# askerlee/AdaFace-dev

Hardware: AMD Instinct MI355X
Metric: denoise-steps/sec SD-1.5 U-Net 512px bs=4/GPU (higher is better)
Workload: dtype f16

## Files before the change

adaface-dev_amd/csrc/af_gemm3.hip:

```cpp
#include <stdlib.h>

#include <algorithm>

#include "af_common.h"

int af_gemm_n_major(int M, int N, int K, int cin);

namespace {

struct Gemm3Dev {
  const half_t* a1;
  const half_t* a2;
  const half_t* wt;
  const half_t* zeros;
  const float* bias;
  const half_t* rowbias;
  const half_t* residual;
  half_t* out;
  half_t* out2;
  int split_col, ld_out2;
  int M, N, K, kpad, npad;
  int c1, c2, lda1, lda2;
  const half_t* a3;
  const half_t* a4;
// ... 1333 lines not shown
  };

#ifdef AF_CONV3H_GN_PROBE
  const float probe_r = 1.0f + p.ln_eps, probe_s = p.ln_eps;
  auto gn_probe_piece = [&](int j, int buf_off, int u) {
    if (wave + NW * j < NP) {
      char* q = af_smem + buf_off + (wave + NW * j) * 1024 + lane * 16;
      const half8_t v = *reinterpret_cast<const half8_t*>(q);
      const int ch = ((u * 64) & 255) + (int)(chunk16 >> 1);
      const floatx4 g0 = *reinterpret_cast<const floatx4*>(p.bias + ch), g1 = *reinterpret_cast<const floatx4*>(p.bias + ch + 4);
      half8_t o;
#pragma unroll
      for (int e = 0; e < 8; ++e) {
        const float y = af_silu(fmaf((float)v[e] * (e < 4 ? g0[e] : g1[e - 4]), probe_r, probe_s));
        o[e] = a_pix[j] >= 0 ? (half_t)y : (half_t)0.f;
      }
      *reinterpret_cast<half8_t*>(q) = o;
    }
  };
#define CHD_GN_PROBE(TAP) if (!last && (TAP) >= 1 && (TAP) - 1 < APW) gn_probe_piece((TAP) >= 1 ? (TAP) - 1 : 0, nbuf, u + 1);
#else
#define CHD_GN_PROBE(TAP)
#endif
  floatx4 acc[TN][TM];
#pragma unroll
  for (int tn = 0; tn < TN; ++tn)
#pragma unroll
    for (int tm = 0; tm < TM; ++tm) acc[tn][tm] = floatx4{0.f, 0.f, 0.f, 0.f};
  const int fr = lane & 15, fq = lane >> 4;
  const int wr0 = WBASE + (wn * TN * 16) * 128 + fr * 128 + ((fq ^ (fr >> 1)) * 16);
  int fa[9][TM];
#pragma unroll
  for (int tm = 0; tm < TM; ++tm) {
    const int q = wm * 64 + tm * 16 + fr;
    const int r = fdiv(q, inv_wd), im = fdiv(r, inv_hi);
    const int hpb = im * blk_px + (r - im * Hi) * Wh + (q - r * Wd);
#pragma unroll
    for (int tap = 0; tap < 9; ++tap) {
      const int hp = hpb + (tap / 3) * Wh + (tap % 3);
      fa[tap][tm] = hp * 128 + ((fq ^ (hp & 7)) * 16);
    }
  }

  if (p.wpf > 0 && p.splits == 1)
    af_prefetch_weight_tile(p.wt, p.kpad, p.npad, tile_n * BN, BN, 0, p.kpad >> 6, p.wpf_coop, tile_m % p.wpf_coop, p.wpf, NW, wave, lane, af_smem + WBASE + 2 * WSZ);

  const int grp = wave >> 2;
  half8_t wf[TN], xf[TM], wf1[TN], xf1[TM];
  auto mfmas = [&]() {
#pragma unroll
    for (int tn = 0; tn < TN; ++tn)
#pragma unroll
      for (int tm = 0; tm < TM; ++tm)
        acc[tn][tm] = __builtin_amdgcn_mfma_f32_16x16x32_f16(wf[tn], xf[tm], acc[tn][tm], 0, 0, 0);
#pragma unroll
    for (int tn = 0; tn < TN; ++tn)
#pragma unroll
      for (int tm = 0; tm < TM; ++tm)
        acc[tn][tm] = __builtin_amdgcn_mfma_f32_16x16x32_f16(wf1[tn], xf1[tm], acc[tn][tm], 0, 0, 0);
  };
#define CHD_READ_FRAGS(TAP)                                                                                                      \
  {                                                                                                                              \
    constexpr int wsl_ = ((TAP) % 3) * WSZ;                                                                                   \
    _Pragma("unroll") for (int tn = 0; tn < TN; ++tn) wf[tn] = *reinterpret_cast<const half8_t*>(af_smem + wr0 + wsl_ + tn * 2048);               \
    _Pragma("unroll") for (int tm = 0; tm < TM; ++tm) xf[tm] = *reinterpret_cast<const half8_t*>(af_smem + fa[TAP][tm]);                            \
    _Pragma("unroll") for (int tn = 0; tn < TN; ++tn) wf1[tn] = *reinterpret_cast<const half8_t*>(af_smem + (wr0 ^ 64) + wsl_ + tn * 2048);         \
    _Pragma("unroll") for (int tm = 0; tm < TM; ++tm) xf1[tm] = *reinterpret_cast<const half8_t*>(af_smem + (fa[TAP][tm] ^ 64));                    \
  }

  __builtin_amdgcn_s_setprio(1);
  const int nchunks = ce - cb;
  if (nchunks > 0) {
    const half_t* src;
    int ld2;
    chunk_src(cb, src, ld2);
#pragma unroll
    for (int j = 0; j < APW; ++j) issue_halo_piece(j, src, ld2, 0);
    issue_w(cb, 0, 0);
    issue_w(cb, 1, 1);
  }
  asm volatile("s_waitcnt vmcnt(0)" ::: "memory");
#ifdef AF_CONV3H_GN_PROBE
  if (nchunks > 0) {
#pragma unroll
    for (int j = 0; j < APW; ++j) gn_probe_piece(j, 0, cb);
  }
#endif
#pragma unroll
  for (int j = 0; j < APW; ++j)
    if (wave + NW * j < NP && a_pix[j] < 0) {
      char* z = af_smem + (wave + NW * j) * 1024 + lane * 16;
      *reinterpret_cast<uintx4_t*>(z) = uintx4_t{0u, 0u, 0u, 0u};
      *reinterpret_cast<uintx4_t*>(z + CH_ASZ) = uintx4_t{0u, 0u, 0u, 0u};
    }
  asm volatile("s_waitcnt lgkmcnt(0)" ::: "memory");
  __builtin_amdgcn_s_barrier();
  __builtin_amdgcn_sched_barrier(0);

  if (grp == 0) {
#pragma nounroll
    for (int u = cb; u < ce; ++u) {
      const bool first = u == cb, last = u + 1 == ce;
      const half_t* hsrc = a1r;
      int hld2 = 0;
      if (!last) chunk_src(u + 1, hsrc, hld2);
      const int nbuf = ((u + 1 - cb) & 1) * CH_ASZ;
#define CHD_STAGE0(TAP)                                                                                                          \
      {                                                                                                                          \
        CHD_READ_FRAGS(TAP)                                                                                                      \
        if (!(first && (TAP) == 0) && !(last && (TAP) == 8)) issue_w((TAP) < 8 ? u : u + 1, ((TAP) + 1) % 9, ((TAP) + 1) % 3);   \
        if (!last && (TAP) < APW) issue_halo_piece((TAP) < APW ? (TAP) : 0, hsrc, hld2, nbuf);                                   \
        CHD_GN_PROBE(TAP)                                                                                                        \
        asm volatile("s_waitcnt lgkmcnt(0)" ::: "memory");                                                                       \
        __builtin_amdgcn_sched_barrier(0);                                                                                       \
        __builtin_amdgcn_s_barrier();                                                                                            \
        __builtin_amdgcn_sched_barrier(0);                                                                                       \
        __builtin_amdgcn_s_setprio(0);                                                                                           \
        mfmas();                                                                                                                 \
        __builtin_amdgcn_s_setprio(1);                                                                                           \
        asm volatile("s_waitcnt vmcnt(0)" ::: "memory");                                                                         \
        __builtin_amdgcn_sched_barrier(0);                                                                                       \
        __builtin_amdgcn_s_barrier();                                                                                            \
        __builtin_amdgcn_sched_barrier(0);                                                                                       \
      }
      CHD_STAGE0(0) CHD_STAGE0(1) CHD_STAGE0(2) CHD_STAGE0(3) CHD_STAGE0(4) CHD_STAGE0(5) CHD_STAGE0(6) CHD_STAGE0(7) CHD_STAGE0(8)
#undef CHD_STAGE0
      const int d = ((u - cb) & 1) ? -CH_ASZ : CH_ASZ;
#pragma unroll
      for (int tap = 0; tap < 9; ++tap)
#pragma unroll
        for (int tm = 0; tm < TM; ++tm) fa[tap][tm] += d;
    }
    __builtin_amdgcn_s_barrier();
  } else {
#pragma nounroll
    for (int u = cb; u < ce; ++u) {
      const bool first = u == cb, last = u + 1 == ce;
      const half_t* hsrc = a1r;
      int hld2 = 0;
      if (!last) chunk_src(u + 1, hsrc, hld2);
      const int nbuf = ((u + 1 - cb) & 1) * CH_ASZ;
#define CHD_STAGE1(TAP)                                                                                                          \
      {                                                                                                                          \
        if (!(first && (TAP) == 0)) {                                                                                            \
          __builtin_amdgcn_s_setprio(0);                                                                                         \
          mfmas();                                                                                                               \
          __builtin_amdgcn_s_setprio(1);                                                                                         \
        }                                                                                                                        \
        asm volatile("s_waitcnt vmcnt(0)" ::: "memory");                                                                         \
        __builtin_amdgcn_sched_barrier(0);                                                                                       \
        __builtin_amdgcn_s_barrier();                                                                                            \
        __builtin_amdgcn_sched_barrier(0);                                                                                       \
        CHD_READ_FRAGS(TAP)                                                                                                      \
        if (!(last && (TAP) >= 7)) issue_w((TAP) < 7 ? u : u + 1, ((TAP) + 2) % 9, ((TAP) + 2) % 3);                             \
        if (!last && (TAP) < APW) issue_halo_piece((TAP) < APW ? (TAP) : 0, hsrc, hld2, nbuf);                                   \
        CHD_GN_PROBE(TAP)                                                                                                        \
        asm volatile("s_waitcnt lgkmcnt(0)" ::: "memory");                                                                       \
        __builtin_amdgcn_sched_barrier(0);                                                                                       \
        __builtin_amdgcn_s_barrier();                                                                                            \
        __builtin_amdgcn_sched_barrier(0);                                                                                       \
      }
      CHD_STAGE1(0) CHD_STAGE1(1) CHD_STAGE1(2) CHD_STAGE1(3) CHD_STAGE1(4) CHD_STAGE1(5) CHD_STAGE1(6) CHD_STAGE1(7) CHD_STAGE1(8)
#undef CHD_STAGE1
      const int d = ((u - cb) & 1) ? -CH_ASZ : CH_ASZ;
#pragma unroll
      for (int tap = 0; tap < 9; ++tap)
#pragma unroll
        for (int tm = 0; tm < TM; ++tm) fa[tap][tm] += d;
    }
    if (nchunks > 0) {
      __builtin_amdgcn_s_setprio(0);
      mfmas();
      __builtin_amdgcn_s_setprio(1);
    }
    asm volatile("s_waitcnt vmcnt(0)" ::: "memory");
    __builtin_amdgcn_s_barrier();
  }
#undef CHD_READ_FRAGS
#undef CHD_GN_PROBE
  if (TAIL && tail_here) {
    int tb = 0;
#pragma unroll
    for (int j = 0; j < 4; ++j) issue_tail_piece(j, 0, tb);
    issue_wk(9 * Cin, 0);
    int ft[TM];
#pragma unroll
    for (int tm = 0; tm < TM; ++tm) ft[tm] = (wm * 64 + tm * 16 + fr) * 128 + ((fq ^ (fr & 7)) * 16);
#pragma nounroll
    for (int t = 0; t < ntail; ++t) {
      asm volatile("s_waitcnt vmcnt(0)" ::: "memory");
      __builtin_amdgcn_s_barrier();
      const int tn_ = tb == 0 ? CH_ASZ : 0;
      if (t + 1 < ntail) {
#pragma unroll
        for (int j = 0; j < 4; ++j) issue_tail_piece(j, t + 1, tn_);
        issue_wk(9 * Cin + (t + 1) * 64, (t + 1) % 3);
      }
      const int ws = (t % 3) * WSZ;
#pragma unroll
      for (int tn = 0; tn < TN; ++tn) wf[tn] = *reinterpret_cast<const half8_t*>(af_smem + wr0 + ws + tn * 2048);
#pragma unroll
      for (int tm = 0; tm < TM; ++tm) xf[tm] = *reinterpret_cast<const half8_t*>(af_smem + tb + ft[tm]);
#pragma unroll
      for (int tn = 0; tn < TN; ++tn) wf1[tn] = *reinterpret_cast<const half8_t*>(af_smem + (wr0 ^ 64) + ws + tn * 2048);
#pragma unroll
      for (int tm = 0; tm < TM; ++tm) xf1[tm] = *reinterpret_cast<const half8_t*>(af_smem + tb + (ft[tm] ^ 64));
      __builtin_amdgcn_s_setprio(0);
      mfmas();
      __builtin_amdgcn_s_setprio(1);
      tb = tn_;
    }
    asm volatile("s_waitcnt vmcnt(0)" ::: "memory");
    __builtin_amdgcn_s_barrier();
  }
  __builtin_amdgcn_s_setprio(0);
  gemm3_epilogue<E3_STD, NWM, NWN, TN, CH_LDS, PATCH>(p, acc, af_smem, tile_m, tile_n, wm, wn, fr, fq, tid);
}

static int conv3h_variant(const af_gemm_desc* d) {
  if (d->taps != 9 || (d->upsample != 0 && d->upsample != 1) || d->tap_shift || d->c1 % 64 != 0 || d->c2 % 64 != 0) return 0;
  const bool n160 = d->N % CH_BN == 0;
  if (!n160 && d->N % 128 != 0) return 0;
  if (d->c3 || d->c4) {
    if (!n160 || d->c3 <= 0 || d->c3 % 64 != 0 || d->c4 < 0 || d->c4 % 64 != 0 || d->a3 == nullptr || (d->c4 > 0 && d->a4 == nullptr) || d->upsample) return 0;
    if ((long)d->M * std::max(d->lda3 ? d->lda3 : d->c3, d->lda4 ? d->lda4 : d->c4) * 2 >= (1L << 32)) return 0;
  }
  const int up = d->upsample ? 2 : 1;
  if ((d->stride ? d->stride : 1) != 1 || d->Ho != up * d->H || d->Wo != up * d->W) return 0;
  if (d->M % CH_BM != 0 || d->M != d->B * d->Ho * d->Wo) return 0;
  if (d->act == AF_ACT_GEGLU || d->out_mode == AF_OUT_SPLIT_T || d->ln_colsum != nullptr || d->kpad % 64 != 0) return 0;
  if ((long)d->B * d->H * d->W * std::max(d->c1, d->c2) * 2 >= (1L << 32)) return 0;
  if (d->Wo > 64) {
    if (n160 || d->Wo % 16 != 0 || d->Ho % 16 != 0 || d->c3 || d->c4) return 0;
    return 3;
  }
  if (d->Wo != 8 && d->Wo != 16 && d->Wo != 32 && d->Wo != 64) return 0;
  const int rows = CH_BM / d->Wo;
  if (d->Ho % rows != 0 && rows % d->Ho != 0) return 0;
  if (d->Ho < rows && (rows / d->Ho) * (d->Ho + 2) * (d->Wo + 2) > CH_NP_MAX * 8) return 0;
  return n160 ? 1 : 2;
}
static bool conv3h_eligible(const af_gemm_desc* d) { return conv3h_variant(d) != 0; }

static int conv3h_chunks(const af_gemm_desc* d) { return (d->c1 + d->c2) / 64; }

static bool launch_conv3h(const Gemm3Dev& p0, hipStream_t stream, bool r5_loop, int variant) {
  Gemm3Dev p = p0;
  p.tiles_n = p.N / (variant == 1 ? CH_BN : 128);
  p.tiles_m = p.M / CH_BM;
  p.patch_tx = p.Wo / 16;
  p.patch_tpi = p.patch_tx * (p.Ho / 16);
  {
    static const int coop_env = getenv("AF_GEMM3_WPF_COOP") ? atoi(getenv("AF_GEMM3_WPF_COOP")) : 32;
    p.wpf_coop = p.tiles_m < coop_env ? p.tiles_m : coop_env;
    if (p.wpf > AF_WPF_MAX) p.wpf = AF_WPF_MAX;
  }
  if (p.counters && (p.splits <= 1 || p.splits > 4 || p.tiles_m * p.tiles_n > AF_SPLITK_MAX_TILES)) p.counters = nullptr;
  p.n_major = af_gemm_n_major(p.M, p.N, p.K, p.c1 + p.c2);
  dim3 grid(p.tiles_m * p.tiles_n, p.splits), block(512);
  if (variant >= 2) {
    static bool set_2 = false, set_3 = false;
    if (variant == 2) {
      if (af_allow_dyn_lds(reinterpret_cast<const void*>(&af_conv3hd_kernel<false, 4, false>), CH_LDS, set_2, "af_gemm"))
        hipLaunchKernelGGL((af_conv3hd_kernel<false, 4, false>), grid, block, CH_LDS, stream, p);
    } else if (af_allow_dyn_lds(reinterpret_cast<const void*>(&af_conv3hd_kernel<false, 4, true>), CH_LDS, set_3, "af_gemm")) {
      hipLaunchKernelGGL((af_conv3hd_kernel<false, 4, true>), grid, block, CH_LDS, stream, p);
    }
    return p.counters != nullptr;
  }
#define AF_CONV3H_CASE(A)                                                                                                                     \
  case A: {                                                                                                                                   \
    static bool set_ = false;                                                                                                                 \
    if (af_allow_dyn_lds(reinterpret_cast<const void*>(&af_conv3h_kernel<A>), CH_LDS, set_, "af_gemm"))                                       \
      hipLaunchKernelGGL(af_conv3h_kernel<A>, grid, block, CH_LDS, stream, p);                                                                \
    break;                                                                                                                                    \
  }
  static const bool diet_env = !(getenv("AF_CONV3H_DIET") && atoi(getenv("AF_CONV3H_DIET")) == 0);
  static const bool diet_dynamic = getenv("AF_GEMM3_ABLATE_DYNAMIC") != nullptr;
  const bool diet = diet_dynamic ? !(getenv("AF_CONV3H_DIET") && atoi(getenv("AF_CONV3H_DIET")) == 0) : diet_env;
  if ((diet || p.c3 > 0) && !r5_loop && (p.ablate & 63) == 0) {
    static bool set_d = false, set_t = false;
    if (p.c3 > 0) {
      if (af_allow_dyn_lds(reinterpret_cast<const void*>(&af_conv3hd_kernel<true>), CH_LDS, set_t, "af_gemm"))
        hipLaunchKernelGGL(af_conv3hd_kernel<true>, grid, block, CH_LDS, stream, p);
    } else if (af_allow_dyn_lds(reinterpret_cast<const void*>(&af_conv3hd_kernel<false>), CH_LDS, set_d, "af_gemm")) {
      hipLaunchKernelGGL(af_conv3hd_kernel<false>, grid, block, CH_LDS, stream, p);
    }
    return p.counters != nullptr;
  }
  switch (p.ablate & 63) {
#ifdef AF_CONV3H_ABLATIONS
    AF_CONV3H_CASE(1) AF_CONV3H_CASE(2) AF_CONV3H_CASE(3) AF_CONV3H_CASE(4) AF_CONV3H_CASE(7) AF_CONV3H_CASE(8) AF_CONV3H_CASE(16) AF_CONV3H_CASE(17) AF_CONV3H_CASE(18) AF_CONV3H_CASE(19) AF_CONV3H_CASE(32)
#endif
    default:
    AF_CONV3H_CASE(0)
  }
#undef AF_CONV3H_CASE
  return p.counters != nullptr;
}

constexpr int FF_C = 320, FF_BM = 128, FF_HC = 64;
constexpr int FF_XS = 5 * FF_BM * 128, FF_W1S = 2 * FF_HC * 128, FF_W2B = FF_C * 128;
constexpr int FF_LDS = FF_XS + 2 * FF_W1S + FF_W2B + FF_BM * 8;

struct FfDev {
  const half_t* x;
  const half_t* w1;
  const float* b1;
  const float* cs1;
  int ln_on;
  const half_t* w2;
  const half_t* zeros;
  int M, inner, kpad1, kpad2;
  float ln_eps;
  Gemm3Dev epi;
  const half_t* wp;
  int kpad_p;
  Gemm3Dev epi_p;
};

template <bool TAILP>
__global__ __launch_bounds__(512, 1) void af_ff320_kernel(FfDev p) {
  constexpr int NW = 8, NWM = 2, TM = 4;
  extern __shared__ __attribute__((aligned(16))) char af_smem[];
  char* Xs = af_smem;
  char* W1r = af_smem + FF_XS;
  char* W2b = W1r + 2 * FF_W1S;
  float* st = reinterpret_cast<float*>(W2b + FF_W2B);
  const int tid = threadIdx.x, lane = tid & 63;
  const int wave = __builtin_amdgcn_readfirstlane(tid >> 6);
  const int wm = wave % NWM, wn = wave / NWM;
  const int tile_m = blockIdx.x;
  const int prow = lane >> 3, slot = lane & 7;
  const int fr = lane & 15, fq = lane >> 4;
  const int rd0 = fr * 128 + (((0 * 4 + fq) ^ (fr >> 1)) * 16);
  const int rd1 = fr * 128 + (((1 * 4 + fq) ^ (fr >> 1)) * 16);
  const int nchunk = p.inner / FF_HC;

  {
    const int coop = gridDim.x < 32 ? gridDim.x : 32;
    af_prefetch_weight_tile(p.w1, p.kpad1, 2 * p.inner, 0, 2 * p.inner, 0, FF_C / 64, coop, tile_m % coop, 1, NW, wave, lane, af_smem + FF_LDS);
    af_prefetch_weight_tile(p.w2, p.kpad2, FF_C, 0, FF_C, 0, p.inner / 64, coop, tile_m % coop, 1, NW, wave, lane, af_smem + FF_LDS);
  }

#pragma unroll
  for (int c = 0; c < 5; ++c)
#pragma unroll
    for (int j = 0; j < 2; ++j) {
      const int row = (wave * 2 + j) * 8 + prow;
      const int m = tile_m * FF_BM + row;
      const int lc = slot ^ ((row >> 1) & 7);
      const half_t* g = m < p.M ? p.x + (size_t)m * FF_C + c * 64 + lc * 8 : p.zeros;
      glds16(g, Xs + c * (FF_BM * 128) + (wave * 2 + j) * 1024);
    }
  auto issue_w1 = [&](int g) {
    const int jc = g / 5, sc = g - jc * 5;
    char* dst = W1r + (g & 1) * FF_W1S;
#pragma unroll
    for (int j = 0; j < 2; ++j) {
      const int row = (wave * 2 + j) * 8 + prow;
      const int lc = slot ^ ((row >> 1) & 7);
      glds16(p.w1 + (size_t)(jc * 2 * FF_HC + row) * p.kpad1 + sc * 64 + lc * 8, dst + (wave * 2 + j) * 1024);
    }
  };
  auto issue_w2 = [&](int jc) {
#pragma unroll
    for (int j = 0; j < 5; ++j) {
      const int row = (wave * 5 + j) * 8 + prow;
      const int lc = slot ^ ((row >> 1) & 7);
      glds16(p.w2 + (size_t)row * p.kpad2 + jc * 64 + lc * 8, W2b + (wave * 5 + j) * 1024);
    }
  };
  issue_w1(0);
  asm volatile("s_waitcnt vmcnt(2)" ::: "memory");
  __builtin_amdgcn_s_barrier();

  {
    const half2_t one2 = {(half_t)1.0f, (half_t)1.0f};
    float s = 0.f, q = 0.f;
    const char* row = Xs + (wave * 16) * 128;
#pragma unroll
    for (int c = 0; c < 5; ++c) {
      const half8_t f0 = *reinterpret_cast<const half8_t*>(row + c * (FF_BM * 128) + rd0), f1 = *reinterpret_cast<const half8_t*>(row + c * (FF_BM * 128) + rd1);
#pragma unroll
      for (int e = 0; e < 8; e += 2) {
        const half2_t a = {f0[e], f0[e + 1]}, b = {f1[e], f1[e + 1]};
        s = __builtin_amdgcn_fdot2(a, one2, s, false);
        q = __builtin_amdgcn_fdot2(a, a, q, false);
        s = __builtin_amdgcn_fdot2(b, one2, s, false);
        q = __builtin_amdgcn_fdot2(b, b, q, false);
      }
    }
    s += __shfl_xor(s, 16, 64);
    q += __shfl_xor(q, 16, 64);
    s += __shfl_xor(s, 32, 64);
    q += __shfl_xor(q, 32, 64);
    if (fq == 0) {
      const float mean = s * (1.0f / FF_C), var = fmaxf(q * (1.0f / FF_C) - mean * mean, 0.f);
      st[2 * (wave * 16 + fr)] = p.ln_on ? mean : 0.f;
      st[2 * (wave * 16 + fr) + 1] = p.ln_on ? rsqrtf(var + p.ln_eps) : 1.f;
    }
  }
  __syncthreads();
  float mean[TM], rstd[TM];
#pragma unroll
  for (int tm = 0; tm < TM; ++tm) {
    const int row = wm * 64 + tm * 16 + fr;
    mean[tm] = st[2 * row];
    rstd[tm] = st[2 * row + 1];
  }

  floatx4 acc2[5][TM];
#pragma unroll
  for (int tn = 0; tn < 5; ++tn)
#pragma unroll
    for (int tm = 0; tm < TM; ++tm) acc2[tn][tm] = floatx4{0.f, 0.f, 0.f, 0.f};

  for (int jc = 0; jc < nchunk; ++jc) {
    floatx4 acc1[2][TM];
#pragma unroll
    for (int tn = 0; tn < 2; ++tn)
#pragma unroll
      for (int tm = 0; tm < TM; ++tm) acc1[tn][tm] = floatx4{0.f, 0.f, 0.f, 0.f};
    const int nv = jc * 2 * FF_HC + wn * 32 + 4 * fq;
    floatx4 bv, bg, cv, cg;
#pragma unroll
    for (int sc = 0; sc < 5; ++sc) {
      const int g = jc * 5 + sc;
      if (sc == 1) asm volatile("s_waitcnt vmcnt(5)" ::: "memory");
      else asm volatile("s_waitcnt vmcnt(0)" ::: "memory");
      __builtin_amdgcn_s_barrier();
      if (g + 1 < nchunk * 5) issue_w1(g + 1);
      if (sc == 0) {
        bv = *reinterpret_cast<const floatx4*>(p.b1 + nv);
        bg = *reinterpret_cast<const floatx4*>(p.b1 + nv + 16);
        cv = *reinterpret_cast<const floatx4*>(p.cs1 + nv);
        cg = *reinterpret_cast<const floatx4*>(p.cs1 + nv + 16);
        issue_w2(jc);
      }
      const char* As = Xs + sc * (FF_BM * 128);
      const char* Ws = W1r + (g & 1) * FF_W1S;
#pragma unroll
      for (int kk = 0; kk < 2; ++kk) {
        const int rd = kk ? rd1 : rd0;
        half8_t wf[2], xf[TM];
#pragma unroll
        for (int tn = 0; tn < 2; ++tn) wf[tn] = *reinterpret_cast<const half8_t*>(Ws + (wn * 32 + tn * 16) * 128 + rd);
#pragma unroll
        for (int tm = 0; tm < TM; ++tm) xf[tm] = *reinterpret_cast<const half8_t*>(As + (wm * 64 + tm * 16) * 128 + rd);
#pragma unroll
        for (int tn = 0; tn < 2; ++tn)
#pragma unroll
          for (int tm = 0; tm < TM; ++tm) acc1[tn][tm] = __builtin_amdgcn_mfma_f32_16x16x32_f16(wf[tn], xf[tm], acc1[tn][tm], 0, 0, 0);
      }
    }
    __builtin_amdgcn_s_barrier();
    {
      char* G = W1r + ((jc * 5 + 4) & 1) * FF_W1S;
#pragma unroll
      for (int tm = 0; tm < TM; ++tm) {
        const int row = wm * 64 + tm * 16 + fr;
        half4_t h;
#pragma unroll
        for (int e = 0; e < 4; ++e) {
          const float xv = rstd[tm] * (acc1[0][tm][e] - mean[tm] * cv[e]) + bv[e];
          const float gv = rstd[tm] * (acc1[1][tm][e] - mean[tm] * cg[e]) + bg[e];
          h[e] = (half_t)(xv * af_gelu_erf(gv));
        }
        const int sl = (wn * 2 + (fq >> 1)) ^ ((row >> 1) & 7);
        *reinterpret_cast<half4_t*>(G + row * 128 + sl * 16 + (fq & 1) * 8) = h;
      }
    }
    asm volatile("s_waitcnt vmcnt(2)" ::: "memory");
    __syncthreads();
    {
      const char* G = W1r + ((jc * 5 + 4) & 1) * FF_W1S;
#pragma unroll
      for (int kk = 0; kk < 2; ++kk) {
        const int rd = kk ? rd1 : rd0;
        half8_t wf[5], xf[TM];
#pragma unroll
        for (int tn = 0; tn < 5; ++tn) wf[tn] = *reinterpret_cast<const half8_t*>(W2b + (wn * 80 + tn * 16) * 128 + rd);
#pragma unroll
        for (int tm = 0; tm < TM; ++tm) xf[tm] = *reinterpret_cast<const half8_t*>(G + (wm * 64 + tm * 16) * 128 + rd);
#pragma unroll
        for (int tn = 0; tn < 5; ++tn)
#pragma unroll
          for (int tm = 0; tm < TM; ++tm) acc2[tn][tm] = __builtin_amdgcn_mfma_f32_16x16x32_f16(wf[tn], xf[tm], acc2[tn][tm], 0, 0, 0);
      }
    }
  }
  if constexpr (!TAILP) {
    gemm3_epilogue<E3_STD, 2, 4, 5, FF_XS + 2 * FF_W1S + FF_W2B>(p.epi, acc2, af_smem, tile_m, 0, wm, wn, fr, fq, tid, nullptr);
  } else {
    constexpr int PST = 160 * 128;
    static_assert(3 * PST <= 2 * FF_W1S + FF_W2B, "the three-slot W_p ring lives in the W1 ring + W2 tile area");
    auto issue_wp = [&](int sidx) {
      const int nh = sidx >= 5 ? 1 : 0, kc = sidx - 5 * nh;
      char* dst = W1r + (sidx % 3) * PST;
#pragma unroll
      for (int j = 0; j < 3; ++j) {
        const int pc = wave + NW * j;
        if (pc < 20) {
          const int row = pc * 8 + prow;
          const int lc = slot ^ ((row >> 1) & 7);
          glds16(p.wp + (size_t)(nh * 160 + row) * p.kpad_p + kc * 64 + lc * 8, dst + pc * 1024);
        }
      }
    };
    __syncthreads();
    issue_wp(0);
    issue_wp(1);
#pragma unroll
    for (int tm = 0; tm < TM; ++tm) {
      const int row = wm * 64 + tm * 16 + fr, m = tile_m * FF_BM + row;
#pragma unroll
      for (int tn = 0; tn < 5; ++tn) {
        const int c = wn * 80 + tn * 16 + 4 * fq;
        floatx4 v = acc2[tn][tm];
        half4_t o = {(half_t)0.f, (half_t)0.f, (half_t)0.f, (half_t)0.f};
        if (m < p.M) {
          if (p.epi.bias) {
            const floatx4 bv = *reinterpret_cast<const floatx4*>(p.epi.bias + c);
#pragma unroll
            for (int e = 0; e < 4; ++e) v[e] += bv[e];
          }
          if (p.epi.residual) {
            const half4_t rv = *reinterpret_cast<const half4_t*>(p.epi.residual + (size_t)m * FF_C + c);
#pragma unroll
            for (int e = 0; e < 4; ++e) v[e] += (float)rv[e];
          }
          o = half4_t{(half_t)v[0], (half_t)v[1], (half_t)v[2], (half_t)v[3]};
        }
        *reinterpret_cast<half4_t*>(Xs + (c >> 6) * (FF_BM * 128) + row * 128 + ((((c & 63) >> 3) ^ ((row >> 1) & 7)) * 16) + ((c >> 2) & 1) * 8) = o;
      }
    }
    floatx4 acc3[5][TM];
#pragma unroll
    for (int tn = 0; tn < 5; ++tn)
#pragma unroll
      for (int tm = 0; tm < TM; ++tm) acc3[tn][tm] = floatx4{0.f, 0.f, 0.f, 0.f};
#pragma nounroll
    for (int sidx = 0; sidx < 10; ++sidx) {
      if (sidx == 9) asm volatile("s_waitcnt vmcnt(0) lgkmcnt(0)" ::: "memory");
      else if (wave < 4) asm volatile("s_waitcnt vmcnt(3) lgkmcnt(0)" ::: "memory");
      else asm volatile("s_waitcnt vmcnt(2) lgkmcnt(0)" ::: "memory");
      __builtin_amdgcn_s_barrier();
      if (sidx + 2 < 10) issue_wp(sidx + 2);
      const int nh = sidx >= 5 ? 1 : 0, kc = sidx - 5 * nh;
      if ((wn >> 1) == nh) {
        const char* Ws = W1r + (sidx % 3) * PST;
        const char* As = Xs + kc * (FF_BM * 128);
#pragma unroll
        for (int kk = 0; kk < 2; ++kk) {
          const int rd = kk ? rd1 : rd0;
          half8_t wf[5], xf[TM];
#pragma unroll
          for (int tn = 0; tn < 5; ++tn) wf[tn] = *reinterpret_cast<const half8_t*>(Ws + ((wn & 1) * 80 + tn * 16) * 128 + rd);
#pragma unroll
          for (int tm = 0; tm < TM; ++tm) xf[tm] = *reinterpret_cast<const half8_t*>(As + (wm * 64 + tm * 16) * 128 + rd);
#pragma unroll
          for (int tn = 0; tn < 5; ++tn)
#pragma unroll
            for (int tm = 0; tm < TM; ++tm) acc3[tn][tm] = __builtin_amdgcn_mfma_f32_16x16x32_f16(wf[tn], xf[tm], acc3[tn][tm], 0, 0, 0);
        }
      }
    }
    gemm3_epilogue<E3_STD, 2, 4, 5, FF_XS + 2 * FF_W1S + FF_W2B>(p.epi_p, acc3, af_smem, tile_m, 0, wm, wn, fr, fq, tid, nullptr);
  }
}

}

extern "C" int af_gemm_halo_variant(const af_gemm_desc* d) { return d != nullptr ? conv3h_variant(d) : 0; }

int af_gemm3_try_launch(const af_gemm_desc* d, int splits, int wide, hipStream_t stream) {
  const bool geglu = d->act == AF_ACT_GEGLU, split_t = d->out_mode == AF_OUT_SPLIT_T;
  const bool halo_r5 = wide == 16;
  if (halo_r5) wide = 11;
  const int halo_variant = wide == 11 ? conv3h_variant(d) : 0;
  if (wide == 11 && halo_variant == 0) return 1;
  if (halo_r5 && (d->c3 > 0 || halo_variant != 1)) return 1;
  if (halo_variant == 3 && splits > 1) return 1;
  if (d->upsample && !((wide == 4 || wide == 5 || (wide >= 8 && wide <= 12)) && d->upsample == 1 && d->taps == 9)) return 1;
  if (d->c1 % BK3 != 0 || d->c2 % BK3 != 0 || d->zeros == nullptr) return 1;
  if (d->c3 > 0 && (wide < 4 || (wide > 10 && wide != 12 && wide != 11) || d->taps != 9 || d->upsample || (d->stride != 0 && d->stride != 1))) return 1;
  if ((geglu || split_t) && (d->taps != 1 || splits > 1)) return 1;
  if (geglu && (!wide || d->N % (wide == 5 ? 128 : 256) != 0)) return 1;
  if (!geglu && wide == 1 && d->N % 320 != 0) return 1;
  if (wide >= 4) {
    if (d->c1 % 64 != 0 || d->c2 % 64 != 0 || d->kpad % 64 != 0) return 1;
    if (wide == 4 && (geglu ? d->N % 256 != 0 : d->N % 320 != 0)) return 1;
    if (wide == 5 && geglu && d->N % 128 != 0) return 1;
    if (wide == 6 && (!geglu || d->N % 320 != 0)) return 1;
    if (wide == 7 && (!geglu || d->N % 256 != 0)) return 1;
    if ((wide == 8 || wide == 10) && (geglu || split_t || d->N % 160 != 0)) return 1;
    if (wide == 9 && (geglu || split_t)) return 1;
    if (wide == 12 && (geglu || split_t || d->N % 128 != 0)) return 1;
    if (wide == 13 && (geglu || d->N % 128 != 0 || d->c3 > 0)) return 1;
    if (wide == 14 && (geglu || d->N % 64 != 0 || d->c3 > 0)) return 1;
    if (wide > 14) return 1;
  }
  if (wide == 2 && (d->N % 256 != 0 || d->taps != 1 || split_t || splits > 1)) return 1;
  if (wide == 3 && (d->N % 320 != 0 || d->taps != 1 || split_t || splits > 1)) return 1;
  if (d->ln_colsum != nullptr && (wide < 4 || d->taps != 1 || d->c2 != 0 || splits > 1)) return 1;
  if (d->gn_partials != nullptr && !((wide == 4 || wide == 8 || wide == 10 || wide == 11) && !geglu && !split_t && splits <= 1)) return 1;
  Gemm3Dev p;
  bool fused = false;
  p.ln_cs = (const float*)d->ln_colsum;
  p.ln_eps = d->ln_eps;
  p.a1 = (const half_t*)d->a1;
  p.a2 = (const half_t*)d->a2;
  p.wt = (const half_t*)d->wt;
  p.zeros = (const half_t*)d->zeros;
  p.bias = (const float*)d->bias;
  p.rowbias = (const half_t*)d->rowbias;
  p.residual = (const half_t*)d->residual;
  p.out = (half_t*)d->out;
  p.out2 = (half_t*)d->out2;
  p.split_col = d->split_col;
  p.ld_out2 = d->ld_out2;
  p.M = d->M;
  p.N = d->N;
  p.K = d->K;
  p.kpad = d->kpad;
  p.npad = (d->N + 127) / 128 * 128;
  p.c1 = d->c1;
  p.c2 = d->c2;
  p.lda1 = d->lda1 ? d->lda1 : d->c1;
  p.lda2 = d->lda2 ? d->lda2 : d->c2;
  p.gn_ws = (float*)d->gn_partials;
  p.gn_cpg = d->gn_cpg;
  p.a3 = (const half_t*)d->a3;
  p.a4 = (const half_t*)d->a4;
  p.c3 = d->c3;
  p.c4 = d->c4;
  p.lda3 = d->lda3 ? d->lda3 : d->c3;
  p.lda4 = d->lda4 ? d->lda4 : d->c4;
  p.H = d->H;
  p.W = d->W;
  p.Ho = d->Ho;
  p.Wo = d->Wo;
  p.HoWo = d->Ho * d->Wo;
  p.stride = d->stride ? d->stride : 1;
  p.upsample = d->upsample;
  p.rows_per_batch = d->rows_per_batch > 0 ? d->rows_per_batch : d->M;
  p.ld_rowbias = d->ld_rowbias;
  p.act = d->act == AF_ACT_SILU ? 1 : (d->act == AF_ACT_QUICKGELU ? 3 : 0);
  p.ld_out = d->ld_out ? d->ld_out : (geglu ? d->N / 2 : (split_t ? d->split_col : d->N));
  p.tiles_n = 0;
  const int nk = p.kpad / BK3;
  p.splits = splits > 1 ? splits : 1;
  if (p.splits > nk) p.splits = nk;
  p.kt_per_split = (nk + p.splits - 1) / p.splits;
  p.splits = (nk + p.kt_per_split - 1) / p.kt_per_split;
  p.ws = (float*)d->workspace;
  p.counters = (d->splitk_fused && d->workspace && d->workspace_bytes > AF_SPLITK_COUNTER_BYTES)
                   ? reinterpret_cast<int*>(static_cast<char*>(d->workspace) + d->workspace_bytes - AF_SPLITK_COUNTER_BYTES) : nullptr;
  static const int wpf_env = getenv("AF_GEMM3_WPREFETCH") ? atoi(getenv("AF_GEMM3_WPREFETCH")) : 4;
  static const bool wpf_dynamic = getenv("AF_GEMM3_ABLATE_DYNAMIC") != nullptr;
  p.wpf = wpf_dynamic ? (getenv("AF_GEMM3_WPREFETCH") ? atoi(getenv("AF_GEMM3_WPREFETCH")) : 4) : wpf_env;
  p.wpf_coop = 1;
  static const int ablate = getenv("AF_GEMM3_ABLATE") ? atoi(getenv("AF_GEMM3_ABLATE")) : 0;
  static const bool ablate_dynamic = getenv("AF_GEMM3_ABLATE_DYNAMIC") != nullptr;
  p.ablate = ablate_dynamic ? (getenv("AF_GEMM3_ABLATE") ? atoi(getenv("AF_GEMM3_ABLATE")) : 0) : ablate;
  {
    const long ldmax = std::max(std::max((long)(d->lda1 ? d->lda1 : d->c1), (long)(d->lda2 ? d->lda2 : d->c2)), std::max((long)(d->lda3 ? d->lda3 : d->c3), (long)(d->lda4 ? d->lda4 : d->c4)));
    if (wide >= 4 && wide != 11 && (long)d->M * ldmax * 2 >= (1L << 32)) return 1;
  }
  {
    const int ncols = geglu ? d->N / 2 : d->N;
    p.stage_ok = ncols % 8 == 0 && p.ld_out % 8 == 0 && (reinterpret_cast<uintptr_t>(p.out) & 15) == 0;
  }
  if (wide == 11) {
    const int nchunk = conv3h_chunks(d);
    p.splits = splits > 1 ? splits : 1;
    if (p.splits > nchunk) p.splits = nchunk;
    p.kt_per_split = (nchunk + p.splits - 1) / p.splits;
    p.splits = (nchunk + p.kt_per_split - 1) / p.kt_per_split;
    if (halo_variant == 3) {
      if (!p.stage_ok) return 1;
      p.splits = 1;
    }
    fused = launch_conv3h(p, stream, halo_r5, halo_variant);
    return (p.splits > 1 && !fused) ? 2 : 0;
  }
  if (wide >= 4) {
    const int nk64 = p.kpad / 64;
    p.splits = splits > 1 ? splits : 1;
    if (p.splits > nk64) p.splits = nk64;
    p.kt_per_split = (nk64 + p.splits - 1) / p.splits;
    p.splits = (nk64 + p.kt_per_split - 1) / p.kt_per_split;
    if (wide == 4) {
      if (geglu) fused = launch3w<1, 2, 4, 4, E3_GEGLU>(p, stream);
      else if (split_t) fused = launch3w<1, 2, 4, 5, E3_SPLIT_T>(p, stream);
      else if (d->taps == 9) fused = launch3w<9, 2, 4, 5>(p, stream);
      else fused = launch3w<1, 2, 4, 5>(p, stream);
    } else if (wide == 5) {
      if (geglu) fused = launch3w<1, 2, 2, 4, E3_GEGLU>(p, stream);
      else if (split_t) fused = launch3w<1, 2, 2, 4, E3_SPLIT_T>(p, stream);
      else if (d->taps == 9) fused = launch3w<9, 2, 2, 4>(p, stream);
      else fused = launch3w<1, 2, 2, 4>(p, stream);
    } else if (wide == 8) {
      if (d->taps == 9) fused = launch3w<9, 2, 2, 5>(p, stream); else fused = launch3w<1, 2, 2, 5>(p, stream);
    } else if (wide == 9) {
      if (d->taps == 9) fused = launch3w<9, 2, 2, 4, E3_STD, 4>(p, stream); else fused = launch3w<1, 2, 2, 4, E3_STD, 4>(p, stream);
    } else if (wide == 12) {
      if (d->taps == 9) fused = launch3w<9, 4, 2, 4>(p, stream); else fused = launch3w<1, 4, 2, 4>(p, stream);
    } else if (wide == 13) {
      if (split_t) fused = launch3w<1, 1, 4, 2, E3_SPLIT_T>(p, stream);
      else if (d->taps == 9) fused = launch3w<9, 1, 4, 2>(p, stream); else fused = launch3w<1, 1, 4, 2>(p, stream);
    } else if (wide == 14) {
      if (split_t) fused = launch3w<1, 2, 2, 2, E3_SPLIT_T>(p, stream);
      else if (d->taps == 9) fused = launch3w<9, 2, 2, 2>(p, stream); else fused = launch3w<1, 2, 2, 2>(p, stream);
    } else if (wide == 10) {
      if (d->taps == 9) fused = launch3w<9, 2, 2, 5, E3_STD, 4>(p, stream); else fused = launch3w<1, 2, 2, 5, E3_STD, 4>(p, stream);
    } else {
      if (wide == 6) fused = launch3w<1, 4, 2, 10, E3_GEGLU>(p, stream); else fused = launch3w<1, 4, 2, 8, E3_GEGLU>(p, stream);
    }
    return (p.splits > 1 && !fused) ? 2 : 0;
  }
  if (wide == 2) {
    if (geglu) fused = launch3<1, 4, 2, 8, E3_GEGLU>(p, stream); else fused = launch3<1, 4, 2, 8>(p, stream);
  } else if (wide == 3) {
    if (geglu) fused = launch3<1, 4, 2, 10, E3_GEGLU>(p, stream); else fused = launch3<1, 4, 2, 10>(p, stream);
  } else if (geglu) {
    fused = launch3<1, 2, 4, 4, E3_GEGLU>(p, stream);
  } else if (split_t) {
    if (wide) fused = launch3<1, 2, 4, 5, E3_SPLIT_T>(p, stream); else fused = launch3<1, 2, 2, 4, E3_SPLIT_T>(p, stream);
  } else if (wide) {
    if (d->taps == 9) fused = launch3<9, 2, 4, 5>(p, stream); else fused = launch3<1, 2, 4, 5>(p, stream);
  } else {
    if (d->taps == 9) fused = launch3<9, 2, 2, 4>(p, stream); else fused = launch3<1, 2, 2, 4>(p, stream);
  }
  return (p.splits > 1 && !fused) ? 2 : 0;
}

int af_gemm3_effective_splits(const af_gemm_desc* d, int splits, int wide) {
  if (wide == 16) wide = 11;
  const int nk = (wide == 11 && conv3h_eligible(d)) ? conv3h_chunks(d) : d->kpad / (wide >= 4 ? 64 : BK3);
  int s = splits > 1 ? splits : 1;
  if (s > nk) s = nk;
  const int per = (nk + s - 1) / s;
  return (nk + per - 1) / per;
}

extern "C" int af_ff_fused(const void* x, const void* w1, const void* b1, const void* ln_colsum, float ln_eps, int kpad1, const void* w2, const void* b2,
                           int kpad2, const void* residual, void* out, int M, int C, int inner, const void* zeros, void* stream) {
  AF_REQUIRE(x && w1 && b1 && w2 && out && zeros, "af_ff_fused: null pointer");
  AF_SUPPORTED(C == FF_C, "af_ff_fused: built for C = 320 (the 64 x 64 level of SD-1.5)");
  AF_REQUIRE(M > 0 && inner > 0 && inner % FF_HC == 0, "af_ff_fused: inner must be a positive multiple of 64");
  AF_REQUIRE(kpad1 >= C && kpad1 % 64 == 0 && kpad2 >= inner && kpad2 % 64 == 0, "af_ff_fused: weight row strides must be 64-multiples covering K");
  FfDev p{};
  p.x = (const half_t*)x;
  p.w1 = (const half_t*)w1;
  p.b1 = (const float*)b1;
  p.cs1 = ln_colsum ? (const float*)ln_colsum : (const float*)b1;
  p.ln_on = ln_colsum != nullptr;
  p.w2 = (const half_t*)w2;
  p.zeros = (const half_t*)zeros;
  p.M = M;
  p.inner = inner;
  p.kpad1 = kpad1;
  p.kpad2 = kpad2;
  p.ln_eps = ln_eps;
  Gemm3Dev& e = p.epi;
  e = Gemm3Dev{};
  e.bias = (const float*)b2;
  e.residual = (const half_t*)residual;
  e.out = (half_t*)out;
  e.M = M;
  e.N = C;
  e.K = inner;
  e.ld_out = C;
  e.splits = 1;
  e.rows_per_batch = M;
  e.stage_ok = (reinterpret_cast<uintptr_t>(out) & 15) == 0;
  AfLaunchScope scope(AF_FAM_GEMM, stream);
  static bool attr_set = false;
  const bool lds_ok = af_allow_dyn_lds(reinterpret_cast<const void*>(&af_ff320_kernel<false>), FF_LDS + AF_WPF_DUMP_BYTES, attr_set, "af_gemm");
  if (lds_ok) hipLaunchKernelGGL(af_ff320_kernel<false>, dim3((M + FF_BM - 1) / FF_BM), dim3(512), FF_LDS + AF_WPF_DUMP_BYTES, (hipStream_t)stream, p);
  return af_check_launch("af_ff_fused");
}

extern "C" int af_ff_chain(const void* x, const void* w1, const void* b1, const void* ln_colsum, float ln_eps, int kpad1, const void* w2, const void* b2, int kpad2,
                           const void* residual, const void* wp, const void* bp, int kpad_p, const void* x_in, void* out, void* gn_partials, int gn_cpg,
                           int rows_per_batch, int M, int C, int inner, const void* zeros, void* stream) {
  AF_REQUIRE(x && w1 && b1 && w2 && wp && out && zeros, "af_ff_chain: null pointer");
  AF_SUPPORTED(C == FF_C, "af_ff_chain: built for C = 320 (the 64 x 64 level of SD-1.5)");
  AF_REQUIRE(M > 0 && inner > 0 && inner % FF_HC == 0, "af_ff_chain: inner must be a positive multiple of 64");
  AF_REQUIRE(kpad1 >= C && kpad1 % 64 == 0 && kpad2 >= inner && kpad2 % 64 == 0 && kpad_p >= C && kpad_p % 64 == 0, "af_ff_chain: weight row strides must be 64-multiples covering K");
  AF_REQUIRE((((uintptr_t)out | (uintptr_t)residual | (uintptr_t)x_in | (uintptr_t)b2 | (uintptr_t)bp) & 15) == 0, "af_ff_chain: out / residual / x_in / b2 / bp must be 16-byte aligned");
  if (gn_partials != nullptr) {
    AF_REQUIRE(gn_cpg > 0 && gn_cpg % 2 == 0 && C % gn_cpg == 0 && C / gn_cpg <= 32 && rows_per_batch > 0 && rows_per_batch % FF_BM == 0 && M % rows_per_batch == 0 &&
                   rows_per_batch / 128 <= 128,
               "af_ff_chain: gn_partials needs an even gn_cpg dividing C into at most 32 groups and whole 128-row blocks per batch item (at most 128)");
  }
  FfDev p{};
  p.x = (const half_t*)x;
  p.w1 = (const half_t*)w1;
  p.b1 = (const float*)b1;
  p.cs1 = ln_colsum ? (const float*)ln_colsum : (const float*)b1;
  p.ln_on = ln_colsum != nullptr;
  p.w2 = (const half_t*)w2;
  p.zeros = (const half_t*)zeros;
  p.M = M;
  p.inner = inner;
  p.kpad1 = kpad1;
  p.kpad2 = kpad2;
  p.ln_eps = ln_eps;
  p.wp = (const half_t*)wp;
  p.kpad_p = kpad_p;
  p.epi = Gemm3Dev{};
  p.epi.bias = (const float*)b2;
  p.epi.residual = (const half_t*)residual;
  Gemm3Dev& e = p.epi_p;
  e = Gemm3Dev{};
  e.bias = (const float*)bp;
  e.residual = (const half_t*)x_in;
  e.out = (half_t*)out;
  e.M = M;
  e.N = C;
  e.K = C;
  e.ld_out = C;
  e.splits = 1;
  e.rows_per_batch = gn_partials ? rows_per_batch : M;
  e.stage_ok = 1;
  e.gn_ws = (float*)gn_partials;
  e.gn_cpg = gn_cpg;
  AfLaunchScope scope(AF_FAM_GEMM, stream);
  static bool attr_set = false;
  const bool lds_ok = af_allow_dyn_lds(reinterpret_cast<const void*>(&af_ff320_kernel<true>), FF_LDS + AF_WPF_DUMP_BYTES, attr_set, "af_gemm");
  if (lds_ok) hipLaunchKernelGGL(af_ff320_kernel<true>, dim3((M + FF_BM - 1) / FF_BM), dim3(512), FF_LDS + AF_WPF_DUMP_BYTES, (hipStream_t)stream, p);
  return af_check_launch("af_ff_chain");
}
```

Measured before the change: 97.11.

## Stream FF W1 and W2 tiles through a unified three-slot LDS ring

Adds a RING variant of the fused GEGLU feed-forward kernel for the 320-channel level. W1 k-slices and the W2 halves now share a three-slot LDS ring, and the gated activations are staged in a separate buffer. Biases and LN column sums are also loaded into LDS asynchronously instead of as per-thread global loads. The aim is to overlap W2 loading with the W1 GEMM and to cut barrier and wait stalls per inner chunk, at the cost of more LDS and more intricate vmcnt bookkeeping. The ring is on by default and can be disabled with AF_FF_RING=0.

```diff
diff --git a/adaface-dev_amd/csrc/af_gemm3.hip b/adaface-dev_amd/csrc/af_gemm3.hip
--- a/adaface-dev_amd/csrc/af_gemm3.hip
+++ b/adaface-dev_amd/csrc/af_gemm3.hip
@@ -1659,6 +1659,10 @@
 constexpr int FF_C = 320, FF_BM = 128, FF_HC = 64;
 constexpr int FF_XS = 5 * FF_BM * 128, FF_W1S = 2 * FF_HC * 128, FF_W2B = FF_C * 128;
 constexpr int FF_LDS = FF_XS + 2 * FF_W1S + FF_W2B + FF_BM * 8;
+constexpr int FF_RS = 160 * 128, FF_GS = FF_BM * 128;
+constexpr int FF_LDS_RING = FF_XS + 3 * FF_RS + FF_GS + 2 * 2 * FF_HC * 4;
+constexpr int FF_EPI_LDS = FF_XS + 2 * FF_W1S + FF_W2B;
+static_assert(FF_LDS_RING <= 160 * 1024 - AF_WPF_DUMP_BYTES && FF_EPI_LDS <= FF_LDS_RING, "af_ff320_kernel: LDS layout");
 
 struct FfDev {
   const half_t* x;
@@ -1676,14 +1680,17 @@
   Gemm3Dev epi_p;
 };
 
-template <bool TAILP>
+template <bool TAILP, bool RING>
 __global__ __launch_bounds__(512, 1) void af_ff320_kernel(FfDev p) {
   constexpr int NW = 8, NWM = 2, TM = 4;
+  constexpr int LDS_MAIN = RING ? FF_LDS_RING : FF_LDS;
   extern __shared__ __attribute__((aligned(16))) char af_smem[];
   char* Xs = af_smem;
   char* W1r = af_smem + FF_XS;
   char* W2b = W1r + 2 * FF_W1S;
-  float* st = reinterpret_cast<float*>(W2b + FF_W2B);
+  char* Gb = W1r + 3 * FF_RS;
+  const float* Bs = reinterpret_cast<const float*>(Gb + FF_GS);
+  float* st = reinterpret_cast<float*>(RING ? Gb : W2b + FF_W2B);
   const int tid = threadIdx.x, lane = tid & 63;
   const int wave = __builtin_amdgcn_readfirstlane(tid >> 6);
   const int wm = wave % NWM, wn = wave / NWM;
@@ -1696,8 +1703,8 @@
 
   {
     const int coop = gridDim.x < 32 ? gridDim.x : 32;
-    af_prefetch_weight_tile(p.w1, p.kpad1, 2 * p.inner, 0, 2 * p.inner, 0, FF_C / 64, coop, tile_m % coop, 1, NW, wave, lane, af_smem + FF_LDS);
-    af_prefetch_weight_tile(p.w2, p.kpad2, FF_C, 0, FF_C, 0, p.inner / 64, coop, tile_m % coop, 1, NW, wave, lane, af_smem + FF_LDS);
+    af_prefetch_weight_tile(p.w1, p.kpad1, 2 * p.inner, 0, 2 * p.inner, 0, FF_C / 64, coop, tile_m % coop, 1, NW, wave, lane, af_smem + LDS_MAIN);
+    af_prefetch_weight_tile(p.w2, p.kpad2, FF_C, 0, FF_C, 0, p.inner / 64, coop, tile_m % coop, 1, NW, wave, lane, af_smem + LDS_MAIN);
   }
 
 #pragma unroll
@@ -1728,8 +1735,32 @@
       glds16(p.w2 + (size_t)row * p.kpad2 + jc * 64 + lc * 8, W2b + (wave * 5 + j) * 1024);
     }
   };
-  issue_w1(0);
-  asm volatile("s_waitcnt vmcnt(2)" ::: "memory");
+  auto issue_ring = [&](int jc, int t) {
+    char* dst = W1r + ((jc * 7 + t) % 3) * FF_RS;
+    if (t < 5) {
+#pragma unroll
+      for (int j = 0; j < 2; ++j) {
+        const int row = (wave * 2 + j) * 8 + prow;
+        const int lc = slot ^ ((row >> 1) & 7);
+        glds16(p.w1 + (size_t)(jc * 2 * FF_HC + row) * p.kpad1 + t * 64 + lc * 8, dst + (wave * 2 + j) * 1024);
+      }
+    } else {
+#pragma unroll
+      for (int j = 0; j < 3; ++j) {
+        const int pc = j < 2 ? wave + NW * j : 16 + (wave & 3);
+        const int row = pc * 8 + prow;
+        const int lc = slot ^ ((row >> 1) & 7);
+        glds16(p.w2 + (size_t)((t - 5) * 160 + row) * p.kpad2 + jc * 64 + lc * 8, dst + pc * 1024);
+      }
+    }
+  };
+  if constexpr (RING) {
+    issue_ring(0, 0);
+    asm volatile("s_waitcnt vmcnt(2)" ::: "memory");
+  } else {
+    issue_w1(0);
+    asm volatile("s_waitcnt vmcnt(2)" ::: "memory");
+  }
   __builtin_amdgcn_s_barrier();
 
   {
@@ -1758,7 +1789,12 @@
       st[2 * (wave * 16 + fr) + 1] = p.ln_on ? rsqrtf(var + p.ln_eps) : 1.f;
     }
   }
-  __syncthreads();
+  if constexpr (RING) {
+    asm volatile("s_waitcnt lgkmcnt(0)" ::: "memory");
+    __builtin_amdgcn_s_barrier();
+  } else {
+    __syncthreads();
+  }
   float mean[TM], rstd[TM];
 #pragma unroll
   for (int tm = 0; tm < TM; ++tm) {
@@ -1773,6 +1809,86 @@
 #pragma unroll
     for (int tm = 0; tm < TM; ++tm) acc2[tn][tm] = floatx4{0.f, 0.f, 0.f, 0.f};
 
+  if constexpr (RING) {
+#define AF_FF_WAIT(n) asm volatile("s_waitcnt vmcnt(" #n ") lgkmcnt(0)" ::: "memory")
+    auto issue_bias = [&](int jc) {
+      const float* src = (lane < 32 ? p.b1 + lane * 4 : p.cs1 + (lane - 32) * 4) + jc * 2 * FF_HC;
+      glds16(reinterpret_cast<const half_t*>(src), Gb + FF_GS);
+    };
+#pragma nounroll
+    for (int jc = 0; jc < nchunk; ++jc) {
+      floatx4 acc1[2][TM];
+#pragma unroll
+      for (int tn = 0; tn < 2; ++tn)
+#pragma unroll
+        for (int tm = 0; tm < TM; ++tm) acc1[tn][tm] = floatx4{0.f, 0.f, 0.f, 0.f};
+#pragma unroll
+      for (int sc = 0; sc < 5; ++sc) {
+        const int s = jc * 7 + sc;
+        if (sc == 0) AF_FF_WAIT(0);
+        else if (sc == 1) AF_FF_WAIT(3);
+        else if (sc == 4) AF_FF_WAIT(3);
+        else AF_FF_WAIT(2);
+        __builtin_amdgcn_s_barrier();
+        if (sc == 0) {
+          issue_ring(jc, 1);
+          issue_ring(jc, 2);
+          issue_bias(jc);
+        } else {
+          issue_ring(jc, sc + 2);
+        }
+        const char* As = Xs + sc * (FF_BM * 128);
+        const char* Ws = W1r + (s % 3) * FF_RS;
+#pragma unroll
+        for (int kk = 0; kk < 2; ++kk) {
+          const int rd = kk ? rd1 : rd0;
+          half8_t wf[2], xf[TM];
+#pragma unroll
+          for (int tn = 0; tn < 2; ++tn) wf[tn] = *reinterpret_cast<const half8_t*>(Ws + (wn * 32 + tn * 16) * 128 + rd);
+#pragma unroll
+          for (int tm = 0; tm < TM; ++tm) xf[tm] = *reinterpret_cast<const half8_t*>(As + (wm * 64 + tm * 16) * 128 + rd);
+#pragma unroll
+          for (int tn = 0; tn < 2; ++tn)
+#pragma unroll
+            for (int tm = 0; tm < TM; ++tm) acc1[tn][tm] = __builtin_amdgcn_mfma_f32_16x16x32_f16(wf[tn], xf[tm], acc1[tn][tm], 0, 0, 0);
+        }
+      }
+      const int nv = wn * 32 + 4 * fq;
+      const floatx4 bv = *reinterpret_cast<const floatx4*>(Bs + nv), bg = *reinterpret_cast<const floatx4*>(Bs + nv + 16);
+      const floatx4 cv = *reinterpret_cast<const floatx4*>(Bs + 2 * FF_HC + nv), cg = *reinterpret_cast<const floatx4*>(Bs + 2 * FF_HC + nv + 16);
+#pragma unroll
+      for (int tm = 0; tm < TM; ++tm) {
+        const int row = wm * 64 + tm * 16 + fr;
+        half4_t h;
+#pragma unroll
+        for (int e = 0; e < 4; ++e) {
+          const float xv = rstd[tm] * (acc1[0][tm][e] - mean[tm] * cv[e]) + bv[e];
+          const float gv = rstd[tm] * (acc1[1][tm][e] - mean[tm] * cg[e]) + bg[e];
+          h[e] = (half_t)(xv * af_gelu_erf(gv));
+        }
+        const int sl = (wn * 2 + (fq >> 1)) ^ ((row >> 1) & 7);
+        *reinterpret_cast<half4_t*>(Gb + row * 128 + sl * 16 + (fq & 1) * 8) = h;
+      }
+      AF_FF_WAIT(0);
+      __builtin_amdgcn_s_barrier();
+      if (jc + 1 < nchunk) issue_ring(jc + 1, 0);
+      const char* Ws = W1r + ((jc * 7 + 5 + (wn >> 1)) % 3) * FF_RS;
+#pragma unroll
+      for (int kk = 0; kk < 2; ++kk) {
+        const int rd = kk ? rd1 : rd0;
+        half8_t wf[5], xf[TM];
+#pragma unroll
+        for (int tn = 0; tn < 5; ++tn) wf[tn] = *reinterpret_cast<const half8_t*>(Ws + ((wn & 1) * 80 + tn * 16) * 128 + rd);
+#pragma unroll
+        for (int tm = 0; tm < TM; ++tm) xf[tm] = *reinterpret_cast<const half8_t*>(Gb + (wm * 64 + tm * 16) * 128 + rd);
+#pragma unroll
+        for (int tn = 0; tn < 5; ++tn)
+#pragma unroll
+          for (int tm = 0; tm < TM; ++tm) acc2[tn][tm] = __builtin_amdgcn_mfma_f32_16x16x32_f16(wf[tn], xf[tm], acc2[tn][tm], 0, 0, 0);
+      }
+    }
+#undef AF_FF_WAIT
+  } else
   for (int jc = 0; jc < nchunk; ++jc) {
     floatx4 acc1[2][TM];
 #pragma unroll
@@ -1848,10 +1964,10 @@
     }
   }
   if constexpr (!TAILP) {
-    gemm3_epilogue<E3_STD, 2, 4, 5, FF_XS + 2 * FF_W1S + FF_W2B>(p.epi, acc2, af_smem, tile_m, 0, wm, wn, fr, fq, tid, nullptr);
+    gemm3_epilogue<E3_STD, 2, 4, 5, FF_EPI_LDS>(p.epi, acc2, af_smem, tile_m, 0, wm, wn, fr, fq, tid, nullptr);
   } else {
     constexpr int PST = 160 * 128;
-    static_assert(3 * PST <= 2 * FF_W1S + FF_W2B, "the three-slot W_p ring lives in the W1 ring + W2 tile area");
+    static_assert(PST == FF_RS && 3 * PST <= 2 * FF_W1S + FF_W2B, "the three-slot W_p ring lives in the W1 ring + W2 tile area (RING: the ring)");
     auto issue_wp = [&](int sidx) {
       const int nh = sidx >= 5 ? 1 : 0, kc = sidx - 5 * nh;
       char* dst = W1r + (sidx % 3) * PST;
@@ -1923,7 +2039,7 @@
         }
       }
     }
-    gemm3_epilogue<E3_STD, 2, 4, 5, FF_XS + 2 * FF_W1S + FF_W2B>(p.epi_p, acc3, af_smem, tile_m, 0, wm, wn, fr, fq, tid, nullptr);
+    gemm3_epilogue<E3_STD, 2, 4, 5, FF_EPI_LDS>(p.epi_p, acc3, af_smem, tile_m, 0, wm, wn, fr, fq, tid, nullptr);
   }
 }
 
@@ -2102,6 +2218,11 @@
   return (nk + per - 1) / per;
 }
 
+static bool ff_ring() {
+  const char* e = getenv("AF_FF_RING");
+  return !(e && atoi(e) == 0);
+}
+
 extern "C" int af_ff_fused(const void* x, const void* w1, const void* b1, const void* ln_colsum, float ln_eps, int kpad1, const void* w2, const void* b2,
                            int kpad2, const void* residual, void* out, int M, int C, int inner, const void* zeros, void* stream) {
   AF_REQUIRE(x && w1 && b1 && w2 && out && zeros, "af_ff_fused: null pointer");
@@ -2134,9 +2255,15 @@
   e.rows_per_batch = M;
   e.stage_ok = (reinterpret_cast<uintptr_t>(out) & 15) == 0;
   AfLaunchScope scope(AF_FAM_GEMM, stream);
-  static bool attr_set = false;
-  const bool lds_ok = af_allow_dyn_lds(reinterpret_cast<const void*>(&af_ff320_kernel<false>), FF_LDS + AF_WPF_DUMP_BYTES, attr_set, "af_gemm");
-  if (lds_ok) hipLaunchKernelGGL(af_ff320_kernel<false>, dim3((M + FF_BM - 1) / FF_BM), dim3(512), FF_LDS + AF_WPF_DUMP_BYTES, (hipStream_t)stream, p);
+  if (ff_ring()) {
+    static bool attr_set = false;
+    const bool lds_ok = af_allow_dyn_lds(reinterpret_cast<const void*>(&af_ff320_kernel<false, true>), FF_LDS_RING + AF_WPF_DUMP_BYTES, attr_set, "af_gemm");
+    if (lds_ok) hipLaunchKernelGGL((af_ff320_kernel<false, true>), dim3((M + FF_BM - 1) / FF_BM), dim3(512), FF_LDS_RING + AF_WPF_DUMP_BYTES, (hipStream_t)stream, p);
+  } else {
+    static bool attr_set = false;
+    const bool lds_ok = af_allow_dyn_lds(reinterpret_cast<const void*>(&af_ff320_kernel<false, false>), FF_LDS + AF_WPF_DUMP_BYTES, attr_set, "af_gemm");
+    if (lds_ok) hipLaunchKernelGGL((af_ff320_kernel<false, false>), dim3((M + FF_BM - 1) / FF_BM), dim3(512), FF_LDS + AF_WPF_DUMP_BYTES, (hipStream_t)stream, p);
+  }
   return af_check_launch("af_ff_fused");
 }
 
@@ -2186,8 +2313,14 @@
   e.gn_ws = (float*)gn_partials;
   e.gn_cpg = gn_cpg;
   AfLaunchScope scope(AF_FAM_GEMM, stream);
-  static bool attr_set = false;
-  const bool lds_ok = af_allow_dyn_lds(reinterpret_cast<const void*>(&af_ff320_kernel<true>), FF_LDS + AF_WPF_DUMP_BYTES, attr_set, "af_gemm");
-  if (lds_ok) hipLaunchKernelGGL(af_ff320_kernel<true>, dim3((M + FF_BM - 1) / FF_BM), dim3(512), FF_LDS + AF_WPF_DUMP_BYTES, (hipStream_t)stream, p);
+  if (ff_ring()) {
+    static bool attr_set = false;
+    const bool lds_ok = af_allow_dyn_lds(reinterpret_cast<const void*>(&af_ff320_kernel<true, true>), FF_LDS_RING + AF_WPF_DUMP_BYTES, attr_set, "af_gemm");
+    if (lds_ok) hipLaunchKernelGGL((af_ff320_kernel<true, true>), dim3((M + FF_BM - 1) / FF_BM), dim3(512), FF_LDS_RING + AF_WPF_DUMP_BYTES, (hipStream_t)stream, p);
+  } else {
+    static bool attr_set = false;
+    const bool lds_ok = af_allow_dyn_lds(reinterpret_cast<const void*>(&af_ff320_kernel<true, false>), FF_LDS + AF_WPF_DUMP_BYTES, attr_set, "af_gemm");
+    if (lds_ok) hipLaunchKernelGGL((af_ff320_kernel<true, false>), dim3((M + FF_BM - 1) / FF_BM), dim3(512), FF_LDS + AF_WPF_DUMP_BYTES, (hipStream_t)stream, p);
+  }
   return af_check_launch("af_ff_chain");
 }
```

Measured after the change: 97.57, median of 6. About the same (+0.5%).
